# XuehaiPan/mate

Hardware: AMD Instinct MI355X
Metric: env-steps/sec MATE-4v8-9 batch=4096 per GPU (random policy, auto-reset) (higher is better)
Workload: dtype f64; 1 GPU; MATE-4v8-9.yaml batch=4096 envs per GPU, uniform random policy (on-device Philox), fused 256-step launches, restarts every 1 launch(es); global_batch=4096, parallelism=env-shard x1, steps_per_launch=256

## Files before the change

### mate_amd/csrc/device_math.hpp

```cpp
#pragma once
#include <hip/hip_runtime.h>
#include <stdint.h>

namespace mate {

constexpr double kRad2Deg = 180.0 / 3.14159265358979323846;
constexpr double kDeg2Rad = 3.14159265358979323846 / 180.0;
constexpr double kTerrain = 1000.0;
constexpr double kWarehouseRadius = 75.0;
constexpr double kWarehouseCenter = 925.0;
constexpr double kMaxViewingAngle = 180.0;

enum Stream : uint32_t { S_TRANSMIT = 1, S_GOAL = 2, S_ACT_CAM = 3, S_ACT_TGT = 4, S_RESET = 5, S_RESET_VIEW = 6 };

struct U4 { uint32_t x, y, z, w; };

__device__ __forceinline__ U4 philox(uint32_t k0, uint32_t k1, uint32_t c0, uint32_t c1, uint32_t c2, uint32_t c3) {
#pragma unroll
    for (int r = 0; r < 10; ++r) {
        const uint64_t p0 = (uint64_t)0xD2511F53u * c0;
        const uint64_t p1 = (uint64_t)0xCD9E8D57u * c2;
        const uint32_t n0 = (uint32_t)(p1 >> 32) ^ c1 ^ k0;
        const uint32_t n1 = (uint32_t)p1;
        const uint32_t n2 = (uint32_t)(p0 >> 32) ^ c3 ^ k1;
// ... 83 lines not shown
    p = FMA_SCX(p, z, 0xbf9e9ae6fc27006aull); p = FMA_SCX(p, z, 0x3fa2c15b5711927aull); p = FMA_SCX(p, z, 0xbfa59976e82d3ff0ull);
    p = FMA_SCX(p, z, 0x3fa82d5d6ef28734ull); p = FMA_SCX(p, z, 0xbfaae5ce6a214619ull); p = FMA_SCX(p, z, 0x3fae1bb48427b883ull);
    p = FMA_SCX(p, z, 0xbfb110e48b207f05ull); p = FMA_SCX(p, z, 0x3fb3b13657b87036ull); p = FMA_SCX(p, z, 0xbfb745d119378e4full);
    p = FMA_SCX(p, z, 0x3fbc71c717e1913cull); p = FMA_SCX(p, z, 0xbfc2492492376b7dull); p = FMA_SCX(p, z, 0x3fc99999999952ccull);
    p = FMA_SCX(p, z, 0xbfd5555555555523ull);
    double r = fma(t, z * p, t);
    const double half_pi = __longlong_as_double(0x3ff921fb54442d18ll), pi = __longlong_as_double(0x400921fb54442d18ll);
    if (ay > ax) r = half_pi - r;
    if (x < 0.0) r = pi - r;
    if (y == 0.0) r = x < 0.0 ? pi : 0.0;
    return copysign(r, y);
}
__device__ __forceinline__ double atan2_deg(double y, double x) { return atan2_finite(y, x) * kRad2Deg; }
__device__ __forceinline__ double atan2_sector(double y, double x) {
    const double ax = fabs(x), ay = fabs(y);
    const bool steep = ay > ax, back = x < 0.0;
    const double t = div_nz(steep ? ax : ay, steep ? ay : ax);
    const double z = t * t;
    double p = __longlong_as_double(0x3eeba404b5e68a13ll);
    p = FMA_SCX(p, z, 0xbf23e260bd3237f4ull); p = FMA_SCX(p, z, 0x3f4b2bb069efb384ull); p = FMA_SCX(p, z, 0xbf67952daf56de9bull);
    p = FMA_SCX(p, z, 0x3f7d6d43a595c56full); p = FMA_SCX(p, z, 0xbf8c6ea4a57d9582ull); p = FMA_SCX(p, z, 0x3f967e295f08b19full);
    p = FMA_SCX(p, z, 0xbf9e9ae6fc27006aull); p = FMA_SCX(p, z, 0x3fa2c15b5711927aull); p = FMA_SCX(p, z, 0xbfa59976e82d3ff0ull);
    p = FMA_SCX(p, z, 0x3fa82d5d6ef28734ull); p = FMA_SCX(p, z, 0xbfaae5ce6a214619ull); p = FMA_SCX(p, z, 0x3fae1bb48427b883ull);
    p = FMA_SCX(p, z, 0xbfb110e48b207f05ull); p = FMA_SCX(p, z, 0x3fb3b13657b87036ull); p = FMA_SCX(p, z, 0xbfb745d119378e4full);
    p = FMA_SCX(p, z, 0x3fbc71c717e1913cull); p = FMA_SCX(p, z, 0xbfc2492492376b7dull); p = FMA_SCX(p, z, 0x3fc99999999952ccull);
    p = FMA_SCX(p, z, 0xbfd5555555555523ull);
    const double r = fma(t, z * p, t);
    const uint32_t base_hi = steep ? 0x3ff921fbu : (back ? 0x400921fbu : 0u);
    const uint32_t base_lo = (steep || back) ? 0x54442d18u : 0u;
    const double base = __hiloint2double((int)base_hi, (int)base_lo);
    const uint32_t flip = (steep != back) ? 0x80000000u : 0u;
    const double sr = __hiloint2double(__double2hiint(r) ^ (int)flip, __double2loint(r));
    return copysign(base + sr, y);
}

__device__ __forceinline__ void sincos_deg(double deg, double &sn, double &cs) {
    const double x = deg * kDeg2Rad;
    const double k = rint(x * 0.63661977236758134308);
    double r = fma(-k, 1.57079632679489655800e+00, x);
    r = fma(-k, 6.12323399573676603587e-17, r);
    const double z = r * r;
    double ps = 2.81145725434552075980e-15;
    ps = FMA_SC(ps, z, -7.64716373181981647590e-13);
    ps = FMA_SC(ps, z, 1.60590438368216145994e-10);
    ps = FMA_SC(ps, z, -2.50521083854417187751e-08);
    ps = FMA_SC(ps, z, 2.75573192239858906526e-06);
    ps = FMA_SC(ps, z, -1.98412698412698412698e-04);
    ps = FMA_SC(ps, z, 8.33333333333333333333e-03);
    ps = FMA_SC(ps, z, -1.66666666666666666667e-01);
    const double s0 = fma(r * z, ps, r);
    double pc = -1.56192069685862264622e-16;
    pc = FMA_SC(pc, z, 4.77947733238738529744e-14);
    pc = FMA_SC(pc, z, -1.14707455977297247139e-11);
    pc = FMA_SC(pc, z, 2.08767569878680989792e-09);
    pc = FMA_SC(pc, z, -2.75573192239858906526e-07);
    pc = FMA_SC(pc, z, 2.48015873015873015873e-05);
    pc = FMA_SC(pc, z, -1.38888888888888888889e-03);
    pc = FMA_SC(pc, z, 4.16666666666666666667e-02);
    const double c0 = fma(z * z, pc, fma(-0.5, z, 1.0));
    const int q = (int)k & 3;
    const double sa = (q & 1) ? c0 : s0, ca = (q & 1) ? s0 : c0;
    sn = (q & 2) ? -sa : sa;
    cs = ((q + 1) & 2) ? -ca : ca;
}

__device__ __forceinline__ void sincos_deg_f32(double deg, float &sn, float &cs) {
// ... 66 lines not shown
```

### mate_amd/csrc/engine_kernels.hpp

```cpp
#pragma once
#include "device_math.hpp"
#include "instrument.hpp"

namespace mate {

enum Mode : int32_t { MODE_STEP = 0, MODE_STEP_RANDOM = 1, MODE_OBSERVE = 2 };

enum { TI_BOUNTY = 0, TI_FREIGHT = 1, TI_GW = 2, TI_TSTEPS = 3, TI_TRSTEPS = 4, TI_STRIDE = 5 };
enum { EI_REMAINING = 0, EI_AWAITING = 16, EI_DELIVERED = 20, EI_EPSTEP = 21, EI_TICK = 22, EI_EPISODE = 23, EI_DONE = 24, EI_PAD = 25, EI_COUNT = 26 };

struct Params {
    int32_t Nc, Nt, No, NK, NJ;
    int32_t Dc, Dt, cam_elems, tgt_elems;
    int32_t SW, DF, NI, DW;
    int32_t n_sector, n_range, sector_rounds, range_rounds;
    int32_t bit_cc, bit_range, bit_camobs, bit_always, MW;
    int32_t fs_range, fs_camobs, fs_always, fs_shared, nflags;
    int32_t nscratch, sc_cam, sc_tgt, sc_obs;
    int32_t tgt_table_off;
    int32_t kmax, nbucket;
    int32_t max_episode_steps, sparse_reward, num_cargoes_per_target, shuffle, start_with_cargoes, n_high;
    int32_t obs_f64;
    float inv_Nt, inv_NK, inv_NJ, inv_Nc;
    double tau, cam_radius, theta_min, rmax, rot, zoom, area, tgt_step, tgt_sight;
// ... 131 lines not shown
    float *scalars;
    uint32_t *masks;
    int32_t *idle_steps;
    uint32_t *own_masks;
    int32_t *done_count;
    int32_t *done_list;
    int32_t *flag_count;
    int32_t *flag_list;
    int32_t *lut_overflow;
    int32_t lut_defer_above;
    const uint8_t *reset_mask;
    const double *reset_tape;
    int32_t reset_tape_len;
    int32_t *reset_draws;
    double *ep_stats;
    double *sort_scratch;
    uint32_t *dev_tick_ptr;
    int32_t *ctrl;
    long long *phase_clocks;
    int32_t debug_skip;
    int64_t N;
    int32_t mode, act_f64, parity, reset_kind;
    int32_t rollout_steps;
    int32_t freeze_done;
    uint32_t tick;
    uint32_t tick_advance;
    int32_t stagger;
    const double2 *cam_grid, *tgt_grid;
    int32_t n_cam_grid, n_tgt_grid;
    int32_t act_discrete;
    int32_t obs_mode;
    int32_t rotate_prio;
    int32_t store_shifted;
    int32_t pipelined;
    int32_t per_step;
};
constexpr int32_t kDoneTag = 4;

__device__ __forceinline__ void phase_prio(int mode, int phase) {
    if (mode == 0) return;
    const int k = (mode >> (2 * phase)) & 3;
    if (k == 0) __builtin_amdgcn_s_setprio(0);
    else if (k == 1) __builtin_amdgcn_s_setprio(1);
    else if (k == 2) __builtin_amdgcn_s_setprio(2);
    else __builtin_amdgcn_s_setprio(3);
}

__device__ __forceinline__ const Ptrs &kernarg_ptrs(const Ptrs &g) {
    static_assert(alignof(Ptrs) == 8 && sizeof(const Params *) == 8, "g follows pp at byte 8 of the kernel arguments");
#if defined(__HIP_DEVICE_COMPILE__)
    (void)g;
    return *(const Ptrs *)((const char *)__builtin_amdgcn_kernarg_segment_ptr() + 8);
#else
    return g;
#endif
}

__device__ __forceinline__ void wave_sync() {
    __builtin_amdgcn_fence(__ATOMIC_RELEASE, "workgroup", "local");
    __builtin_amdgcn_wave_barrier();
    __builtin_amdgcn_fence(__ATOMIC_ACQUIRE, "workgroup", "local");
}

enum Flow : int {
    FLOW_ANY = 0,
    FLOW_RANDOM = 1,
// ... 520 lines not shown
    overflow = w[0].x != w[0].x;
    double2 k0 = w[0], k1 = w[1];
#pragma unroll
    for (int i = 1; i < kDegSlots - 1; ++i)
        if (w[i].x <= x) { k0 = w[i]; k1 = w[i + 1]; }
    if (k0.x == x) return k0.y;
    const double slope = (k1.y - k0.y) / (k1.x - k0.x);
    double res = slope * (x - k0.x) + k0.y;
    if (res != res) {
        res = slope * (x - k1.x) + k1.y;
        if (res != res && k0.y == k1.y) res = k0.y;
    }
    return res;
}

struct SectorEval { bool seen, need; double rn, x; int64_t lc; };

constexpr int kRoleRounds = 5;
__device__ __forceinline__ float range_rim(float lim) { return lim * (lim * 2e-5f + 2e-3f); }
template <typename ObsT, int L>
__device__ __forceinline__ bool range_exact(const Ctx<ObsT, L> &c, int tj, int j) {
    const double dx = c.ex[tj] - c.ex[j], dy = c.ey[tj] - c.ey[j];
    const double d2 = fma(dy, dy, dx * dx);
    const double lim = c.p.tgt_sight + c.er[j], lim2 = lim * lim;
    if (d2 < lim2 * (1.0 - 1e-14)) return true;
    if (d2 > lim2 * (1.0 + 1e-14)) return false;
    return sqrt_pos(d2) <= lim;
}
typedef __attribute__((address_space(3))) const double lds_cf64;
typedef __attribute__((address_space(3))) const float lds_cf32;
__device__ __forceinline__ uint32_t lds_addr(const void *q) { return (uint32_t)(uintptr_t)(__attribute__((address_space(3))) const char *)q; }
__device__ __forceinline__ double lds_f64(uint32_t a, int byte_off = 0) { return *(lds_cf64 *)(uintptr_t)(a + (uint32_t)byte_off); }
__device__ __forceinline__ float lds_f32(uint32_t a, int byte_off = 0) { return *(lds_cf32 *)(uintptr_t)(a + (uint32_t)byte_off); }
constexpr uint32_t kPass1Diag = 0xfffffffeu, kPass1None = 0xffffffffu;
constexpr int kSectorDiag = -3;
struct RangeRoles {
    uint32_t at[kRoleRounds], aj[kRoleRounds];
    float lim2[kRoleRounds];
    float rim[kRoleRounds];
    int32_t sector;
    uint32_t sec_cam, sec_other, sec_draw;
    uint32_t pass1[2];
    uint32_t block[1 + kRoleRounds];
    uint32_t block_bits;
    float reach2[kRoleRounds];
};
__device__ __forceinline__ void image_block_of(const Params &p, bool viewer_is_camera, int viewer, int j, uint32_t &word, uint32_t &code) {
    int src, col;
    if (j < p.Nc) { src = p.off_pub + 32 * j; code = 3u; }
    else if (j < p.Nc + p.No) { src = p.off_pub + 32 * (p.Nc + p.Nt) + 16 * (j - p.Nc); code = 1u; }
    else { src = p.off_pub + 32 * p.Nc + 32 * (j - p.Nc - p.No); code = 2u; }
    if (viewer_is_camera) {
        col = 22 + (j < p.Nc ? 5 * p.Nt + 4 * p.No + 7 * j : j < p.Nc + p.No ? 5 * p.Nt + 4 * (j - p.Nc) : 5 * (j - p.Nc - p.No));
        word = (uint32_t)src | ((uint32_t)(p.off_img + 4 * (viewer * p.Dc + col)) << 16);
    } else {
        col = 27 + (j < p.Nc ? 7 * j : j < p.Nc + p.No ? 7 * p.Nc + 4 * (j - p.Nc) : 7 * p.Nc + 4 * p.No + 5 * (j - p.Nc - p.No));
        word = (uint32_t)src | ((uint32_t)(p.off_img + 4 * (p.cam_elems + viewer * p.Dt + col)) << 16);
    }
}
__device__ __forceinline__ void pin_roles(RangeRoles &r, int rounds = kRoleRounds, bool image = true, bool sector = true) {
#pragma unroll
    for (int i = 0; i < kRoleRounds; ++i)
        if (i < rounds) { asm volatile("" : "+v"(r.at[i])); asm volatile("" : "+v"(r.aj[i])); asm volatile("" : "+v"(r.lim2[i])); asm volatile("" : "+v"(r.rim[i])); asm volatile("" : "+v"(r.reach2[i])); }
    if (image) {
#pragma unroll
        for (int i = 0; i < 1 + kRoleRounds; ++i)
            if (i <= rounds) asm volatile("" : "+v"(r.block[i]));
        asm volatile("" : "+v"(r.block_bits));
    }
    if (sector) { asm volatile("" : "+v"(r.sector)); asm volatile("" : "+v"(r.sec_cam)); asm volatile("" : "+v"(r.sec_other)); asm volatile("" : "+v"(r.sec_draw)); }
    else { asm volatile("" : "+v"(r.pass1[0])); asm volatile("" : "+v"(r.pass1[1])); }
}
template <typename ObsT>
__device__ __forceinline__ void range_roles(const Ctx<ObsT> &c, RangeRoles &roles) {
    const Params &p = c.p;
    roles.block_bits = 0;
    roles.sector = sector_role(p, (p.sector_rounds - 1) * 64 + c.lane);
#pragma unroll
    for (int round = 0; round < kRoleRounds; ++round) {
        const int q = round * 64 + c.lane;
        const int qq = q < p.n_range ? q : 0;
        const int t = (int)(((float)qq + 0.5f) * p.inv_NJ);
        const int j = qq - t * p.NJ;
        const int tj = c.tgt_slot(t);
        const float lim = (float)(p.tgt_sight + c.er[j]);
        const bool valid = q < p.n_range && round < p.range_rounds;
        roles.at[round] = lds_addr(c.exf + tj); roles.aj[round] = lds_addr(c.exf + j);
        roles.lim2[round] = !valid ? -INFINITY : j == tj ? INFINITY : lim * lim - range_rim(lim);
        roles.rim[round] = !valid ? -INFINITY : j == tj ? INFINITY : lim * lim + range_rim(lim);
        {
            const float step = (float)(((c.capword() >> t) & 1ull) ? p.tgt_step * 0.5 : p.tgt_step);
            const float reach = step + (float)c.er[j] + 1e-3f;
            roles.reach2[round] = (q < p.n_range && round < p.range_rounds && j < p.Nc + p.No) ? reach * reach : -1.0f;
        }
        roles.block[1 + round] = 0u;
        if (c.image() && q < p.n_range && round < p.range_rounds) {
            uint32_t code;
            image_block_of(p, false, t, j, roles.block[1 + round], code);
            roles.block_bits |= code << (2 * (1 + round));
        }
    }
#pragma unroll
    for (int round = 0; round < 2; ++round) {
        const int role = sector_role(p, round * 64 + c.lane);
        roles.pass1[round] = kPass1None;
        if (role >= 0) {
            const int cam = role & 0xff, other = (role >> 8) & 0xff;
            const bool is_target = (role >> 16) & 1;
            roles.pass1[round] = !is_target && cam == other ? kPass1Diag : (uint32_t)(8 * cam) | ((uint32_t)(8 * (is_target ? c.tgt_slot(other) : other)) << 16);
        }
    }
    roles.block[0] = 0u;
    roles.sec_cam = roles.sec_other = roles.sec_draw = lds_addr(c.base);
    if (roles.sector >= 0) {
        const int cam = roles.sector & 0xff, other = (roles.sector >> 8) & 0xff;
        const bool is_target = (roles.sector >> 16) & 1;
        const int oj = is_target ? c.tgt_slot(other) : other;
        if (c.image()) {
            uint32_t code;
            image_block_of(p, true, cam, oj, roles.block[0], code);
            roles.block_bits |= code;
        }
        roles.sec_cam += 8u * (uint32_t)cam; roles.sec_other += 8u * (uint32_t)oj;
        if (is_target) roles.sec_draw += 8u * (uint32_t)(cam * p.Nt + other);
        if (!is_target && cam == other) roles.sector = kSectorDiag;
    }
}

template <typename ObsT>
__device__ __forceinline__ void near_seed(const Ctx<ObsT> &c, const RangeRoles &roles, NearCarry &near) {
#pragma unroll
    for (int round = 0; round < kRoleRounds; ++round) {
        near.w[round] = 0ull;
        if (round < c.p.range_rounds) {
            const float dx = lds_f32(roles.at[round]) - lds_f32(roles.aj[round]);
            const float dy = lds_f32(roles.at[round], 4 * c.p.NJ) - lds_f32(roles.aj[round], 4 * c.p.NJ);
            near.w[round] = __ballot(fmaf(dy, dy, dx * dx) <= roles.reach2[round]);
        }
    }
}

__device__ __forceinline__ int sector_role(const Params &p, int q) {
    if (q < 0 || q >= p.n_sector) return -1;
    int cam, other; bool is_target;
    if (q < p.bit_cc) { cam = (int)(((float)q + 0.5f) * p.inv_Nt); other = q - cam * p.Nt; is_target = true; }
    else { const int r = q - p.bit_cc; cam = (int)(((float)r + 0.5f) * p.inv_Nc); other = r - cam * p.Nc; is_target = false; }
    return cam | (other << 8) | ((int)is_target << 16);
}
constexpr int kNoRole = -2;
__device__ __forceinline__ bool sector_out_of_range(double d2, double s2) {
    if (d2 > s2 * (1.0 + 1e-14)) return true;
    return !(d2 < s2 * (1.0 - 1e-14)) && sqrt_pos(d2) > sqrt_pos(s2);
}
template <bool RANGED = false, typename ObsT, int L>
__device__ __forceinline__ SectorEval sector_eval(Ctx<ObsT, L> &c, int q, uint32_t tick, uint32_t stream, bool predrawn, int role = kNoRole) {
    const Params &p = c.p;
// ... 27 lines not shown
}

template <typename ObsT>
__device__ __forceinline__ SectorEval sector_eval_held(Ctx<ObsT> &c, const RangeRoles &h, uint32_t tick, uint32_t stream, bool predrawn) {
    const Params &p = c.p;
    SectorEval e;
    e.seen = false; e.need = false;
    const int role = h.sector;
    if (role < 0) { e.seen = role == kSectorDiag; return e; }
    const int ent = p.off_ent, yoff = 8 * p.NJ;
    const double rx = lds_f64(h.sec_other, ent) - lds_f64(h.sec_cam, ent), ry = lds_f64(h.sec_other, ent + yoff) - lds_f64(h.sec_cam, ent + yoff);
    const double d2 = fma(ry, ry, rx * rx);
    if (sector_out_of_range(d2, lds_f64(h.sec_cam, p.off_tmp))) return e;
    const double ang = atan2_sector(ry, rx) * kRad2Deg;
    double ra = fabs(lds_f64(h.sec_cam, p.off_dy) - ang);
    const double alt = 360.0 - ra;
    if (alt < ra) ra = alt;
    if (ra * 2.0 > lds_f64(h.sec_cam, p.off_dy + 8 * p.Nc)) return e;
    if (p.No == 0) { e.seen = true; return e; }
    if ((role >> 16) & 1) {
        double u;
        if (predrawn && p.Nc * p.Nt <= c.predrawn_pairs()) u = lds_f64(h.sec_draw, p.off_tmp + 8 * (p.Nc + p.Nt));
        else {
            const int pair = (role & 0xff) * p.Nt + ((role >> 8) & 0xff);
            if (predrawn && pair < c.predrawn_pairs()) u = c.udraw(pair);
            else u = c.draw(tick, stream, (uint32_t)pair);
        }
        if ((p.tau <= 0.5) ? (u > 1.0 - p.tau) : (u <= p.tau)) { e.seen = true; return e; }
    }
    e.need = true; e.rn = d2; e.x = normalize_angle(ang); e.lc = c.env * p.Nc + (role & 0xff);
    return e;
}

template <typename ObsT, int L>
__device__ __forceinline__ void sector_fetch(const Ctx<ObsT, L> &c, const SectorEval &e, double2 (&w)[kDegWords]) {
    if (e.need) {
        const double2 *rec = c.g.lut_deg + (e.lc * kLutCells + degree_of(e.x)) * kDegWords;
#pragma unroll
        for (int i = 0; i < kDegWords; ++i) w[i] = rec[i];
    }
}

template <typename ObsT, int L>
__device__ __forceinline__ bool sector_resolve(const Ctx<ObsT, L> &c, const SectorEval &e, double2 (&w)[kDegWords]) {
    if (!e.need) return e.seen;
    bool overflow;
    double limit = segment_interp(w, e.x, overflow);
    if (overflow) {
        int start = (int)w[0].y, count = (int)w[1].x;
        const double2 *knots = c.g.lut_knots + e.lc * c.p.kmax;
        if (c.pivots && count >= 2 && count <= kPivotKnots && w[1].y > 0.0) {
            const int q = (int)w[1].y, last = count - 1;
            const double pv[8] = {w[2].x, w[2].y, w[3].x, w[3].y, w[4].x, w[4].y, w[5].x, w[5].y};
            int nle = 0;
#pragma unroll
            for (int i = 0; i < 8; ++i) nle += pv[i] <= e.x ? 1 : 0;
            const int base = nle * q;
#pragma unroll
            for (int i = 0; i < kDegSlots; ++i) w[i] = knots[start + (base + i < last ? base + i : last)];
            limit = degree_interp(w, e.x, overflow);
        } else {
        while (count > kQuarterKnots && count <= 4 * 256 + 1) {
            const int q = (count + 2) / 4, last = count - 1;
            const double a1 = knots[start + (q < last ? q : last)].x;
            const double a2 = knots[start + (2 * q < last ? 2 * q : last)].x;
            const double a3 = knots[start + (3 * q < last ? 3 * q : last)].x;
            const int base = e.x >= a3 ? 3 * q : (e.x >= a2 ? 2 * q : (e.x >= a1 ? q : 0));
            start += base;
            count = (q + 1 < count - base) ? q + 1 : count - base;
        }
        if (count >= 2 && count <= kQuarterKnots) {
            const int q = (count + 2) / 4, last = count - 1;
            const double a1 = knots[start + (q < last ? q : last)].x;
            const double a2 = knots[start + (2 * q < last ? 2 * q : last)].x;
            const double a3 = knots[start + (3 * q < last ? 3 * q : last)].x;
            const int base = e.x >= a3 ? 3 * q : (e.x >= a2 ? 2 * q : (e.x >= a1 ? q : 0));
#pragma unroll
            for (int i = 0; i < kDegSlots; ++i) w[i] = knots[start + (base + i < last ? base + i : last)];
            limit = degree_interp(w, e.x, overflow);
        } else {
            limit = lut_lookup(knots, c.g.lut_bucket + e.lc * c.p.nbucket, c.g.lut_count[e.lc], e.x);
        }
        }
    }
    const double lim = limit * (1.0 + 1e-6), lim2 = lim * lim;
    if (e.rn < lim2 * (1.0 - 1e-14)) return lim > 0.0;
    if (e.rn > lim2 * (1.0 + 1e-14)) return false;
    return sqrt_pos(e.rn) <= lim;
}

template <bool HELD, bool COMPACT = false, typename ObsT, int L>
__device__ __forceinline__ void update_view(Ctx<ObsT, L> &c, uint32_t tick, uint32_t stream, bool predrawn, const RangeRoles &held, uint32_t &seen_out,
                                            NearCarry *near_next = nullptr, unsigned long long *sector_ballot = nullptr) {
    const Params &p = c.p;
    const int lane = c.lane;
    seen_out = 0u;
    double2 w[kDegWords];
    int n_cand = 0;
    uint8_t *cand = c.base + p.off_list;
    static_assert(L == 64 || !HELD, "held lane roles: one wave per environment");
    const bool compact = L == 64 && COMPACT && p.sector_rounds >= 2 && p.n_sector <= 256;
#define MATE_N_SR (L == 64 ? p.sector_rounds : c.rounds_of(p.n_sector))
#define MATE_N_RR (L == 64 ? p.range_rounds : c.rounds_of(p.n_range))
    if (compact) {
        for (int round = 0; round < p.sector_rounds; ++round) {
            const int q = round * 64 + lane;
            bool diag = false, in_range = false;
            if (HELD && p.sector_rounds == 2) {
                const uint32_t held_pair = held.pass1[round & 1];
                if (held_pair != kPass1None) {
                    diag = held_pair == kPass1Diag;
                    if (!diag) {
                        const uint32_t a_cam = lds_addr(c.base) + (held_pair & 0xffffu), a_oj = lds_addr(c.base) + (held_pair >> 16);
                        const double rx = lds_f64(a_oj, p.off_ent) - lds_f64(a_cam, p.off_ent), ry = lds_f64(a_oj, p.off_ent + 8 * p.NJ) - lds_f64(a_cam, p.off_ent + 8 * p.NJ);
                        in_range = !sector_out_of_range(fma(ry, ry, rx * rx), lds_f64(a_cam, p.off_tmp));
                    }
                    set_flag(c, q, diag);
                }
            } else {
            const int role = sector_role(p, q);
            if (role >= 0) {
                const int cam = role & 0xff, other = (role >> 8) & 0xff;
                const bool is_target = (role >> 16) & 1;
                diag = !is_target && cam == other;
// ... 86 lines not shown
        write_range_ballots();
        if (lane < n_cand) {
            sector_fetch(c, first, w);
            if (sector_resolve(c, first, w)) { set_flag(c, q_first, true); atomicOr(&c.mask[q_first >> 5], 1u << (q_first & 31)); }
        }
        asm volatile("" :: "v"(touch0), "v"(touch1));
        for (int k = lane + 64; k < n_cand; k += 64) {
            const int q = cand[k];
            const SectorEval e = sector_eval<true>(c, q, tick, stream, predrawn);
            sector_fetch(c, e, w);
            if (sector_resolve(c, e, w)) { set_flag(c, q, true); atomicOr(&c.mask[q >> 5], 1u << (q & 31)); }
        }
    } else {
        const bool both_in_flight = L < 64 && MATE_N_SR == 2 && p.Nc * p.Nt < 16;
        SectorEval early;
        early.seen = false; early.need = false;
        double2 w_early[kDegWords];
        if (both_in_flight) {
            early = sector_eval(c, lane, tick, stream, predrawn);
            sector_fetch(c, early, w_early);
        }
        for (int round = 0; round + 1 < MATE_N_SR && !both_in_flight; ++round) {
            const SectorEval e = sector_eval(c, round * L + lane, tick, stream, predrawn);
            sector_fetch(c, e, w);
            const bool seen = sector_resolve(c, e, w);
            if (round * L + lane < p.n_sector) set_flag(c, round * L + lane, seen);
            const unsigned long long b = c.ballot(seen);
            if constexpr (L == 64) { if (lane == 0) { c.mask[2 * round] = (uint32_t)b; c.mask[2 * round + 1] = (uint32_t)(b >> 32); } }
            else c.put_bits(round * L, b);
        }
        const int last = MATE_N_SR - 1;
        SectorEval pending;
        pending.seen = false; pending.need = false;
        if (last >= 0) {
            if constexpr (HELD) pending = sector_eval_held(c, held, tick, stream, predrawn);
            else pending = sector_eval(c, last * L + lane, tick, stream, predrawn);
            sector_fetch(c, pending, w);
        }
        SUB_STAMP(c, 13);
        range_tests();
        if (both_in_flight) {
            const bool seen = sector_resolve(c, early, w_early);
            if (lane < p.n_sector) set_flag(c, lane, seen);
            c.put_bits(0, c.ballot(seen));
        }
        if (last >= 0) {
            const bool seen = sector_resolve(c, pending, w);
            if (!c.image() && last * L + lane < p.n_sector) set_flag(c, last * L + lane, seen);
            seen_out |= (uint32_t)seen;
            const unsigned long long b = c.ballot(seen);
            if constexpr (L == 64) { if (lane == 0) { c.mask[2 * last] = (uint32_t)b; c.mask[2 * last + 1] = (uint32_t)(b >> 32); } }
            else c.put_bits(last * L, b);
            if (sector_ballot) *sector_ballot = b;
        }
        write_range_ballots();
    }
    SUB_STAMP(c, 14);
    if (!c.statics_done) {
        if (lane < p.Nc) {
            const uint64_t m = c.camobs(lane);
            c.mask[(p.bit_camobs >> 5) + 2 * lane] = (uint32_t)m;
            c.mask[(p.bit_camobs >> 5) + 2 * lane + 1] = (uint32_t)(m >> 32);
        }
        if (lane == 0) { c.mask[p.bit_always >> 5] = 1u; if (!c.image()) set_flag(c, p.fs_always, true); }
        if (!c.image())
        for (int q = lane; q < p.Nc * p.No; q += L) {
            const int cam = (int)(((float)q + 0.5f) * p.inv_No);
            const int o = q - cam * p.No;
            set_flag(c, p.fs_camobs + cam * p.No + o, (c.camobs(cam) >> o) & 1ull);
        }
    }
    if (sector_ballot) return;
    wave_sync();
    if (lane < p.Nt) {
        int any = 0;
        for (int cam = 0; cam < p.Nc; ++cam) any |= (int)c.mask_bit(cam * p.Nt + lane);
        c.tracked(lane) = any;
        const double x = c.tx(lane), y = c.ty(lane);
        const bool px = x > 0.0, py = y > 0.0;
        const double wx = px ? kWarehouseCenter : -kWarehouseCenter, wy = py ? kWarehouseCenter : -kWarehouseCenter;
// ... 1241 lines not shown
    if (blockIdx.x == 0 && threadIdx.x == 0 && g.done_count) g.done_count[g.parity ^ 1] = 0;
    const int wave = __builtin_amdgcn_readfirstlane((int)(threadIdx.x >> 6));
    const int hw_lane = threadIdx.x & 63, lane = hw_lane & (L - 1), shift = hw_lane & ~(L - 1);
    const int slot = E == 1 ? wave : wave * E + (hw_lane >> (E == 8 ? 3 : E == 4 ? 4 : 5));
    const int64_t env = (int64_t)blockIdx.x * (4 * E) + slot;
    if (env >= g.N) return;
    const Ptrs &gk = kernarg_ptrs(g);
    MATE_PROF(const long long t_wave = (long long)__builtin_amdgcn_s_memtime();)
    {
        Ctx<ObsT, L> c(p, gk, smem + slot * p.lds_wave_bytes, lane, env, FLOW_ANY, shift);
        load_records(c);
        wave_sync();
        build_entities(c);
        if (!(E > 1 && g.per_step && !g.freeze_done)) list_finished_at_entry(c);
        wave_sync();
    }
    PROLOGUE_STAMP(8);
    constexpr bool IMAGE = E == 1 && Shape::kImage;
    constexpr bool HOLD_ROLES = E == 1 && Shape::kHoldRoles;
    static_assert(E == 1 || !Shape::kImage, "the row image is a whole-wave mode");
    static_assert(kNearWords == kRoleRounds, "one ballot per range round");
    static_assert(!IMAGE || (Shape::kHoldRoles && sizeof(ObsT) == 4 && FLOW != FLOW_ANY), "row-image mode: f32 rows, held lane roles, a folded flow");
    constexpr int kSubC = (Shape::kChunksC + L - 1) / L, kSubT = (Shape::kChunksT + L - 1) / L;
    constexpr int kGC = E == 1 ? Shape::kHeldGC : (kSubC + kSubT <= 12 ? kSubC : 2), kGT = E == 1 ? Shape::kHeldGT : (kSubC + kSubT <= 12 ? kSubT : 6);
    PackDescriptorsT<kGC, kGT> held;
    if constexpr (!IMAGE) {
        Ctx<ObsT, L> c(p, gk, smem + slot * p.lds_wave_bytes, lane, env, FLOW, shift);
        load_pack_descriptors(c, held);
    }
    RangeRoles roles;
    if constexpr (HOLD_ROLES) {
        Ctx<ObsT> c(p, gk, smem + wave * p.lds_wave_bytes, lane, env, FLOW);
        range_roles(c, roles);
        pin_roles(roles);
        PROLOGUE_STAMP(9);
        if constexpr (IMAGE) image_statics(c);
    }
    PROLOGUE_STAMP(10);
    NearCarry near{};
    if constexpr (HOLD_ROLES) {
        Ctx<ObsT> c(p, gk, smem + wave * p.lds_wave_bytes, lane, env, FLOW);
        near_seed(c, roles, near);
    }
    uint32_t hw_id;
    asm volatile("s_getreg_b32 %0, hwreg(HW_REG_HW_ID)" : "=s"(hw_id));
    const int wave_slot = (int)(hw_id & 15u);
    MATE_PROF(long long acc[8] = {0, 0, 0, 0, 0, 0, 0, 0};
              long long t_prev = (long long)__builtin_amdgcn_s_memtime();
              const long long t_first = t_prev, r_first = (long long)__builtin_amdgcn_s_memrealtime();)
    bool stepped = false;
    int last_gw = -1;
    DrawCarry carry{0u, 0u, 0xffffffffu};
    DrawRole draws_of_lane;
    {
        Ctx<ObsT, L> c(p, gk, smem + slot * p.lds_wave_bytes, lane, env, FLOW, shift);
        draws_of_lane = draw_role(c);
    }
    constexpr bool HELDSTATE = IMAGE && FLOW == FLOW_RANDOM;
    HeldState h{};
    int finished = 0;
    const uint32_t tick0 = (E > 1 ? p.dev_tick : 0u) + g.tick;
    const uint32_t cam_low = (uint32_t)(reinterpret_cast<uintptr_t>(g.cam_obs) >> 4) & 7u, tgt_low = (uint32_t)(reinterpret_cast<uintptr_t>(g.tgt_obs) >> 4) & 7u;
    const int n_steps = g.rollout_steps;
    if constexpr (HELDSTATE) {
        Ctx<ObsT> c(p, gk, smem + wave * p.lds_wave_bytes, lane, env, FLOW);
        held_load(c, h);
        finished = __builtin_amdgcn_readfirstlane((int)(c.ei(EI_DONE) != 0));
    }
    PROLOGUE_STAMP(11);
#pragma clang loop unroll(disable)
    for (int r = 0; r < n_steps; ++r) {
        int lane_r = lane, wave_r = wave, slot_r = slot;
        asm volatile("" : "+v"(lane_r));
        asm volatile("" : "+s"(wave_r));
        if constexpr (E == 1) slot_r = wave_r; else asm volatile("" : "+v"(slot_r));
        const Params *pr = pp;
        asm volatile("" : "+s"(pr));
        const Shape shape_r(pr, true);
        const Params &p = shape_r.get();
        const int64_t env_r = (int64_t)blockIdx.x * (4 * E) + slot_r;
        if constexpr (HOLD_ROLES) pin_roles(roles, p.range_rounds, IMAGE, p.sector_rounds == 1);
        Ctx<ObsT, L> c(p, gk, smem + slot_r * p.lds_wave_bytes, lane_r, env_r, FLOW, shift);
        c.out = (int64_t)r * g.N + env_r;
        c.statics_done = stepped;
        c.pivots = Shape::kGreedyHeld;
        if (HELDSTATE ? finished != 0 : (c.ei(EI_DONE) != 0 && (E == 1 || !g.per_step || g.freeze_done))) {
            if (lane_r == 0 && g.scalars) { float *o = g.scalars + c.out * 8; o[0] = 0.f; o[1] = 0.f; o[2] = 2.f; o[3] = o[4] = o[5] = o[6] = o[7] = 0.f; }
            if (lane_r == 0 && g.idle_steps) g.idle_steps[env_r] += 1;
            continue;
        }
        const uint32_t tick = tick0 + (uint32_t)r;
        if (g.rotate_prio) {
            const int turn = g.rotate_prio >= 8 ? ((int)(__builtin_amdgcn_s_memtime() >> g.rotate_prio) + wave_slot) & 3 : (r + wave_slot) & 3;
            if (turn & 2) { if (turn & 1) __builtin_amdgcn_s_setprio(3); else __builtin_amdgcn_s_setprio(2); }
            else { if (turn & 1) __builtin_amdgcn_s_setprio(1); else __builtin_amdgcn_s_setprio(0); }
        }
        ROLL_STAMP(7);
        StepDraws draws{0.0, 0.0};
        pin_draw_role(draws_of_lane);
        draws = step_draws(c, tick, &carry, &draws_of_lane);
        if constexpr (FLOW == FLOW_ACT_F32) draws = prefetch_action(c);
        ROLL_STAMP(0);
        if constexpr (HELDSTATE) {
            simulate_cameras_held(c, draws, h);
            ROLL_STAMP(1);
            simulate_targets_held(c, draws, near, h);
            ROLL_STAMP(2);
            uint32_t seen = 0u;
            unsigned long long sector_ballot = 0ull;
            update_view<true, true>(c, tick, S_TRANSMIT, true, roles, seen, &near, &sector_ballot);
            bool tracked; int inside;
            view_tail_held(c, sector_ballot, h, tracked, inside);
            ROLL_STAMP(3);
            finished = assign_and_score_held(c, tick, g.scalars, h, tracked, inside);
            ROLL_STAMP(4);
            image_targets_held(c, h, last_gw); image_blocks(c, roles, seen);
            ROLL_STAMP(5);
            image_store(c, cam_low, tgt_low); store_masks(c);
            wave_sync();
            stepped = true;
            ROLL_STAMP(6);
            continue;
        }
        simulate_cameras(c, draws, true);
        ROLL_STAMP(1);
        simulate_targets(c, draws, HOLD_ROLES ? &near : nullptr);
        ROLL_STAMP(2);
        uint32_t seen = 0u;
        update_view<HOLD_ROLES, true>(c, tick, S_TRANSMIT, true, roles, seen, HOLD_ROLES ? &near : nullptr);
        ROLL_STAMP(3);
        assign_and_score(c, tick, g.scalars);
        ROLL_STAMP(4);
        if constexpr (IMAGE) {
            image_targets(c, last_gw); image_blocks(c, roles, seen);
            ROLL_STAMP(5);
            image_store(c, cam_low, tgt_low); store_masks(c);
        } else {
            fill_scratch(c, last_gw);
            ROLL_STAMP(5);
            pack_observations<true, Shape::kGreedyHeld>(c, held);
        }
        wave_sync();
        stepped = true;
// ... 23 lines not shown
```

### mate_amd/csrc/mate_engine.hip

```cpp
#include <hip/hip_runtime.h>
#include <hip/hip_ext.h>

#include <algorithm>
#include <atomic>
#include <cmath>
#include <cstdarg>
#include <cstdio>
#include <cstdlib>
#include <cstring>
#include <map>
#include <mutex>
#include <random>
#include <string>
#include <vector>

#include "../../include/mate_engine.h"
#include "reset_kernels.hpp"
#include "policy_kernels.hpp"
#include "aux_kernels.hpp"
#include "state_rows.hpp"

using namespace mate;

static thread_local std::string g_error;
// ... 31 lines not shown
#include "shape_group.inc"
#undef MATE_SHAPE_GROUP
#define MATE_SHAPE_GROUP 5
#include "shape_group.inc"
#undef MATE_SHAPE_GROUP
#endif

static KernelSet pick_kernels(int Nc, int Nt, int No, bool f64, bool generic, bool no_image) {
    KernelSet k;
    if (!generic && (pick_kernels_group0(Nc, Nt, No, f64, no_image, &k) || pick_kernels_group1(Nc, Nt, No, f64, no_image, &k) ||
                     pick_kernels_group2(Nc, Nt, No, f64, no_image, &k) || pick_kernels_group3(Nc, Nt, No, f64, no_image, &k) ||
                     pick_kernels_group4(Nc, Nt, No, f64, no_image, &k) || pick_kernels_group5(Nc, Nt, No, f64, no_image, &k))) {
        k.specialised = 1;
        return k;
    }
    return f64 ? f64_kernels<AnyShape>() : f32_kernels<AnyShape, void, true>(no_image);
}

struct Switches {
    bool generic = false;
    bool flow_generic = false;
    int stagger = -1;
    int lut_small_cap = 0;
    bool reset_monolithic = false;
    int rollout_rotate = 1;
    bool no_image = false;
    bool policy_split = false;
    int step_split = -1;
    bool zoom_iterate = false;
    bool step_sub_wave = true;
    int sub_wave_mode = 2;
    bool step_greedy_rollout = false;
    bool pipelined_low_priority = true;
    bool pipelined_serial = false;
};
static Switches read_switches() {
    Switches w;
    auto flag = [](const char *name) { const char *v = getenv(name); return v && atoi(v) != 0; };
    w.generic = flag("MATE_GENERIC");
    w.flow_generic = flag("MATE_FLOW_GENERIC");
    if (const char *v = getenv("MATE_STAGGER")) w.stagger = atoi(v);
    if (const char *v = getenv("MATE_LUT_SMALL_CAP")) w.lut_small_cap = atoi(v);
    w.reset_monolithic = flag("MATE_RESET_MONOLITHIC");
    if (const char *v = getenv("MATE_ROLLOUT_ROTATE")) w.rollout_rotate = atoi(v);
    w.zoom_iterate = flag("MATE_ZOOM_ITERATE");
    w.policy_split = flag("MATE_POLICY_SPLIT");
    w.step_greedy_rollout = flag("MATE_STEP_GREEDY_ROLLOUT");
    w.no_image = flag("MATE_NO_IMAGE");
    if (const char *v = getenv("MATE_STEP_SUBWAVE")) w.step_sub_wave = atoi(v) != 0;
    if (const char *v = getenv("MATE_SUBWAVE")) w.sub_wave_mode = atoi(v) == 0 ? 0 : 1;
    if (const char *v = getenv("MATE_STEP_SPLIT")) w.step_split = atoi(v) != 0;
    if (const char *v = getenv("MATE_PIPELINED_PRIORITY")) w.pipelined_low_priority = atoi(v) != 0;
    w.pipelined_serial = flag("MATE_PIPELINED_SERIAL");
    return w;
}

struct mate_engine {
    Switches sw{};
    hipStream_t last_stream = nullptr;
    bool launched = false, multi_stream = false;
    Params p{};
    Params *d_params = nullptr;
    Ptrs g{};
    ResetLds rl{};
    ResetLds rl_small{};
    mate_config cfg{};
    int device = 0;
    int64_t N = 0;
    int parity = 0;
    uint32_t tick = 0;
    int64_t steps_since_reset = 0;
    bool was_reset = false;
    bool dev_tick = false;
    int dev_frames = 1;
    int dev_interval = 1;
    int pending_interval = 0;
    bool pipelined = false;
    int pipe_every = 1, pipe_count = 0;
    hipStream_t side = nullptr;
    hipEvent_t ev_launch = nullptr, ev_reset[2] = {nullptr, nullptr};
    bool reset_in_flight[2] = {false, false};
    size_t step_lds = 0, reset_lds = 0;
    KernelSet k{};
    size_t image_wave_bytes = 0;
    int64_t cus = 256;
    int split_on = 0;
// ... 798 lines not shown
    HIP_TRY(hipGetLastError());
    if (mode == MODE_OBSERVE) return MATE_OK;
    if (!e->dev_tick) e->tick += 1;
    return restart_finished(e, auto_reset, Restart{io, true, RESET_DONE, PH_PLACE | PH_LUT | PH_VIEW, false, e->greedy_team_bits != 0, 1u, kStepFlow}, stream);
}

extern "C" int mate_engine_step(mate_engine *e, const mate_step_io *io, int32_t auto_reset, void *stream) {
    return refresh_state_rows(e, launch_step(e, io, MODE_STEP, auto_reset, (hipStream_t)stream), stream);
}
extern "C" int mate_engine_step_random(mate_engine *e, const mate_step_io *io, int32_t auto_reset, void *stream) {
    return refresh_state_rows(e, launch_step(e, io, MODE_STEP_RANDOM, auto_reset, (hipStream_t)stream), stream);
}
static int sub_wave_of_launch(const mate_engine *e, bool greedy) {
    const int mode = e->sw.sub_wave_mode;
    if (mode == 0 || e->k.sub_wave <= 1 || !(greedy ? (const void *)e->k.rollout_greedy_sub : (const void *)e->k.rollout_sub[0])) return 1;
    if (mode == 1) return e->k.sub_wave;
    if (e->N < 32 * e->cus) return 1;
    if (!greedy && e->p.Nc * e->p.Nt >= 16) return 1;
    return e->k.sub_wave;
}

static int rollout_random_impl(mate_engine *e, const mate_step_io *io, int32_t steps, int32_t auto_reset, void *stream_) {
    if (!e) return fail(MATE_EINVAL, "null engine");
    hipStream_t stream = (hipStream_t)stream_;
    { const int rc_ = enter(e, stream, "rollout"); if (rc_ != MATE_OK) return rc_; }
    if (e->dev_tick) return fail(MATE_ESTATE, "not available while the step counter is device-resident (mate_engine_device_tick)");
    if (steps < 1) return fail(MATE_EINVAL, "rollout needs at least one step");
    note_stream(e, stream);
    { int rc = flush_pending(e, auto_reset, kRolloutFlow, stream); if (rc != MATE_OK) return rc; }
    Ptrs g = e->g;
    apply_io(g, io);
    g.mode = MODE_STEP_RANDOM; g.parity = e->parity; g.reset_kind = -1; g.tick = e->tick; g.rollout_steps = steps;
    g.tape_ct = nullptr; g.tape_goal = nullptr;
    g.rotate_prio = e->sw.rollout_rotate;
    if (auto_reset != 1) g.done_count = nullptr;
    const int E = sub_wave_of_launch(e, false);
    const unsigned blocks = (unsigned)((e->N + 4 * E - 1) / (4 * E));
    Timed t;
    { const int rc_ = take_timing_events(e, true, &t); if (rc_ != MATE_OK) return rc_; }
    const int flow = (!e->sw.flow_generic && !g.act_discrete && g.obs_mode == 0 && !g.xdesc && !g.xab && g.scratch_init &&
                      (g.cam_obs || e->p.Nc == 0) && g.tgt_obs && g.scalars) ? FLOW_RANDOM : FLOW_ANY;
    e->last_flow = flow;
    const StepFn fn = E > 1 ? e->k.rollout_sub[flow] : e->k.rollout[flow];
    const size_t lds = E > 1 ? E * e->step_lds : (flow == FLOW_RANDOM && e->k.image) ? 4 * e->image_wave_bytes : e->step_lds;
    hipExtLaunchKernelGGL(fn, dim3(blocks), dim3(256), lds, stream, t.a, t.b, 0, (const Params *)e->d_params, (const Ptrs)g);
    HIP_TRY(hipGetLastError());
    e->tick += (uint32_t)steps;
    return restart_finished(e, auto_reset, Restart{nullptr, false, RESET_FLAGGED, PH_PLACE | PH_LUT, false, false, 0u, kRolloutFlow}, stream);
}

extern "C" int mate_engine_rollout_random(mate_engine *e, const mate_step_io *io, int32_t steps, int32_t auto_reset, void *stream) {
    return refresh_state_rows(e, rollout_random_impl(e, io, steps, auto_reset, stream), stream);
}

static size_t fused_rollout_lds(const mate_engine *e, int E = 1) { return (size_t)E * (4 * (size_t)e->p.lds_wave_bytes + 4 * (size_t)policy_slice_bytes(e->q.PW, e->p.Nc, e->p.Nt)) + (E == 1 ? 1024 : 0); }
static size_t step_greedy_lds(const mate_engine *e, bool cameras = true) {
    return 4 * (size_t)e->p.lds_wave_bytes + 4 * (size_t)step_greedy_slice_bytes(e->q.PW, e->q.TW, e->p.Nc, e->p.Nt, e->p.MW, cameras);
}
static bool use_step_greedy(const mate_engine *e) { return e->k.step_greedy && !e->sw.step_greedy_rollout && step_greedy_lds(e) <= 160 * 1024; }

static int policy_enable(mate_engine *e) {
    if (e->policy_ready) return MATE_OK;
    const Params &p = e->p;
    PolicyPtrs &q = e->q;
    q.TW = pol_target_words(p.Nt);
    q.PW = pol_record_words(p.Nc, p.Nt);
    q.caller_team = -1;
// ... 117 lines not shown
            int least = 0, greatest = 0;
            HIP_TRY(hipDeviceGetStreamPriorityRange(&least, &greatest));
            if (!e->sw.pipelined_low_priority) HIP_TRY(hipStreamCreateWithFlags(&e->side, hipStreamNonBlocking));
            else HIP_TRY(hipStreamCreateWithPriority(&e->side, hipStreamNonBlocking, least));
        }
        HIP_TRY(hipEventCreateWithFlags(&e->ev_launch, hipEventDisableTiming));
        for (int q = 0; q < 2; ++q) HIP_TRY(hipEventCreateWithFlags(&e->ev_reset[q], hipEventDisableTiming));
    }
    if (pipelined && !e->pipelined) {
        HIP_TRY(hipMemsetAsync(e->g.done_count, 0, 2 * sizeof(int32_t), stream));
        e->reset_in_flight[0] = e->reset_in_flight[1] = false;
        e->pipelined = true;
        e->pipe_every = pipe_every; e->pipe_count = 0;
    }
    Ptrs g = e->g;
    apply_io(g, io);
    g.pipelined = pipelined ? 1 : 0;
    if ((e->p.Nc > 0 && !g.cam_obs) || !g.tgt_obs || !g.scalars) return fail(MATE_EINVAL, "rollout_greedy needs the observation and scalar outputs");
    if (g.obs_mode != 0 || g.xdesc) return fail(MATE_EINVAL, "rollout_greedy packs plain observations (no fused transform / team mode)");
    if (team_caller == 0 && e->p.Nc == 0) return fail(MATE_EINVAL, "the scenario has no cameras to act for");
    if (team_caller >= 0 && !(team_caller == 0 ? g.cam_act : g.tgt_act))
        return fail(MATE_EINVAL, "rollout_versus_greedy needs the %s team's joint action", team_caller == 0 ? "camera" : "target");
    if (team_caller >= 0 && (((g.act_discrete & 1) && team_caller == 0 && !g.cam_grid) || ((g.act_discrete & 2) && team_caller == 1 && !g.tgt_grid)))
        return fail(MATE_ESTATE, "discrete actions passed before mate_engine_set_action_grids");
    const int E = ((!per_step || e->sw.step_sub_wave) && fused_rollout_lds(e, e->k.sub_wave) <= 160 * 1024) ? sub_wave_of_launch(e, true) : 1;
    const bool light = per_step && use_step_greedy(e) && E == 1;
    const PolicyFn fn = light ? e->k.step_greedy : E > 1 ? e->k.rollout_greedy_sub : e->k.rollout_greedy;
    const size_t lds = light ? step_greedy_lds(e, team_caller != 0) : fused_rollout_lds(e, E);
    if (lds > 160 * 1024) return fail(MATE_EINVAL, "rollout_greedy: %zu bytes of LDS per workgroup do not fit", lds);
    g.mode = MODE_STEP; g.reset_kind = -1; g.rollout_steps = steps;
    g.parity = e->dev_tick ? 0 : e->parity;
    g.tick = e->dev_tick ? (uint32_t)e->steps_since_reset * (uint32_t)steps : e->tick;
    g.tape_ct = nullptr; g.tape_goal = nullptr; g.freeze_done = 0;
    g.rotate_prio = e->sw.rollout_rotate;
    if (per_step ? auto_reset == 0 : (auto_reset != 1 && !pipelined)) g.done_count = nullptr;
    if (pipelined && e->reset_in_flight[e->parity]) { HIP_TRY(hipStreamWaitEvent(stream, e->ev_reset[e->parity], 0)); e->reset_in_flight[e->parity] = false; }
    PolicyPtrs q = e->q;
    std::memset(&q.tape, 0, sizeof(q.tape));
    q.caller_team = team_caller;
    const unsigned blocks = (unsigned)((e->N + 4 * E - 1) / (4 * E));
    Timed t;
    { const int rc_ = take_timing_events(e, !e->dev_tick, &t); if (rc_ != MATE_OK) return rc_; }
    e->last_flow = light ? FLOW_STEP_GREEDY : FLOW_GREEDY;
    launch(fn, dim3(blocks), dim3(256), lds, stream, t, e->d_params, g, q);
    HIP_TRY(hipGetLastError());
    if (!e->dev_tick) e->tick += (uint32_t)steps;
    const int full = PH_PLACE | PH_LUT | PH_VIEW;
    if (per_step) return restart_finished(e, auto_reset, Restart{io, false, RESET_DONE, full, false, true, 1u, kStepFlow}, stream);
    if (!pipelined) return restart_finished(e, auto_reset, Restart{nullptr, false, RESET_FLAGGED, full, true, false, (uint32_t)steps, kRolloutFlow}, stream);
    if (++e->pipe_count < e->pipe_every) return MATE_OK;
    e->pipe_count = 0;
    const bool serial = e->sw.pipelined_serial;
    hipStream_t rs = serial ? stream : e->side;
    if (!serial) { HIP_TRY(hipEventRecord(e->ev_launch, stream)); HIP_TRY(hipStreamWaitEvent(rs, e->ev_launch, 0)); }
    Ptrs r = restart_ptrs(e);
    r.pipelined = 1;
    const bool multi_before = e->multi_stream;
    int rc = launch_reset(e, r, RESET_DONE, full, rs, true);
    if (rc != MATE_OK) return rc;
    HIP_TRY(hipMemsetAsync(e->g.done_count + e->parity, 0, sizeof(int32_t), rs));
    if (!serial) { HIP_TRY(hipEventRecord(e->ev_reset[e->parity], rs)); e->reset_in_flight[e->parity] = true; }
    e->last_stream = stream; e->multi_stream = multi_before;
    e->parity ^= 1;
    return MATE_OK;
}

extern "C" int mate_engine_rollout_greedy(mate_engine *e, const mate_step_io *io, int32_t steps, int32_t auto_reset, void *stream) {
// ... 479 lines not shown
```

Measured before the change: 765.8 million env-steps/s.

## Add f32 screening pass for sector visibility with exact f64 fallback on band

Adds a float32 pre-screen for the camera sector visibility test. It uses fast rsq/rcp, an f32 atan2 and tolerance bands to classify each pair as seen, hidden or needing the LUT cell, and runs the exact f64 sector evaluation only when some lane in the wave lands inside an uncertainty band. The aim is to cut f64 atan2/sqrt work and LUT recomputation in the held-roles rollout path. It needs extra pinned registers for the pass1 LDS addresses and adds wave-wide ballots. It also depends on the band margins being wide enough to keep results exact. The path is compiled only when MATE_SECTOR_SCREEN is defined and can be disabled at runtime with MATE_SECTOR_EXACT.

```diff
diff --git a/mate_amd/csrc/device_math.hpp b/mate_amd/csrc/device_math.hpp
--- a/mate_amd/csrc/device_math.hpp
+++ b/mate_amd/csrc/device_math.hpp
@@ -139,6 +139,57 @@
     const uint32_t flip = (steep != back) ? 0x80000000u : 0u;
     const double sr = __hiloint2double(__double2hiint(r) ^ (int)flip, __double2loint(r));
     return copysign(base + sr, y);
+}
+
+constexpr float kSectorShift = 1.74e-4f;
+#if defined(__HIP_DEVICE_COMPILE__)
+__host__ __device__ __forceinline__ float rsq_f32(float x) { return __builtin_amdgcn_rsqf(x); }
+__host__ __device__ __forceinline__ float rcp_f32(float x) { return __builtin_amdgcn_rcpf(x); }
+#else
+__host__ __device__ __forceinline__ float rsq_f32(float x) { return 1.0f / __builtin_sqrtf(x); }
+__host__ __device__ __forceinline__ float rcp_f32(float x) { return 1.0f / x; }
+#endif
+__host__ __device__ __forceinline__ float atan2_deg_f32(float y, float x) {
+    const float ax = __builtin_fabsf(x), ay = __builtin_fabsf(y);
+    const bool steep = ay > ax, back = x < 0.0f;
+    const float t = (steep ? ax : ay) * rcp_f32(steep ? ay : ax);
+    const float z = t * t;
+    float p = 0.0073740179650485516f;
+    p = __builtin_fmaf(p, z, -0.03551992028951645f); p = __builtin_fmaf(p, z, 0.08216780424118042f); p = __builtin_fmaf(p, z, -0.13398802280426025f);
+    p = __builtin_fmaf(p, z, 0.1986185610294342f); p = __builtin_fmaf(p, z, -0.3332539498806f);
+    const float r = __builtin_fmaf(t, z * p, t) * 57.29577951308232f;
+    const float base = steep ? 90.0f : (back ? 180.0f : 0.0f);
+    const float a = (steep != back) ? base - r : base + r;
+    return __builtin_copysignf(a, y);
+}
+__host__ __device__ __forceinline__ float sector_bearing_band(float inv_d) { return __builtin_fmaf(1.25e-2f, inv_d, 2e-4f); }
+__host__ __device__ __forceinline__ int sector_range_screen(float d2f, float df, float s2f) {
+    const float band = __builtin_fmaf(8e-4f, df, __builtin_fmaf(1e-6f, d2f + s2f, 1e-6f));
+    const float diff = d2f - s2f;
+    return diff > band ? 1 : (diff < -band ? -1 : 0);
+}
+__host__ __device__ __forceinline__ int sector_angle_screen(float bearing, float phif, float thetaf, float band) {
+    float ra = __builtin_fabsf(phif - bearing);
+    const float alt = 360.0f - ra;
+    if (alt < ra) ra = alt;
+    const float over = __builtin_fmaf(2.0f, ra, -thetaf), rim = __builtin_fmaf(2.0f, band, 4e-4f);
+    return over > rim ? 1 : (over < -rim ? -1 : 0);
+}
+__host__ __device__ __forceinline__ bool sector_cell_screen(float bearing, float band, int cells_per_degree, int &cell) {
+    const float u = (bearing + 180.0f) * (float)cells_per_degree;
+    const float fl = __builtin_floorf(u), fr = u - fl, rim = __builtin_fmaf((float)cells_per_degree, band, 1e-4f);
+    int c = (int)fl;
+    const int last = 360 * cells_per_degree - 1;
+    c = c < 0 ? 0 : (c > last ? last : c);
+    cell = c;
+    return fr > rim && 1.0f - fr > rim;
+}
+__host__ __device__ __forceinline__ int sector_limit_screen(float df, float limf, float slopef, float lead, float band) {
+    const float lim = limf * 1.000001f;
+    const float rim = __builtin_fmaf(__builtin_fabsf(slopef), band, __builtin_fmaf(1e-6f, df + limf, 4e-4f));
+    if (!(lead >= band)) return 0;
+    const float diff = df - lim;
+    return diff > rim ? 1 : (diff < -rim ? -1 : 0);
 }
 
 __device__ __forceinline__ void sincos_deg(double deg, double &sn, double &cs) {
diff --git a/mate_amd/csrc/engine_kernels.hpp b/mate_amd/csrc/engine_kernels.hpp
--- a/mate_amd/csrc/engine_kernels.hpp
+++ b/mate_amd/csrc/engine_kernels.hpp
@@ -187,6 +187,7 @@
     int32_t obs_mode;
     int32_t rotate_prio;
     int32_t store_shifted;
+    int32_t sector_exact;
     int32_t pipelined;
     int32_t per_step;
 };
@@ -773,6 +774,11 @@
 __device__ __forceinline__ uint32_t lds_addr(const void *q) { return (uint32_t)(uintptr_t)(__attribute__((address_space(3))) const char *)q; }
 __device__ __forceinline__ double lds_f64(uint32_t a, int byte_off = 0) { return *(lds_cf64 *)(uintptr_t)(a + (uint32_t)byte_off); }
 __device__ __forceinline__ float lds_f32(uint32_t a, int byte_off = 0) { return *(lds_cf32 *)(uintptr_t)(a + (uint32_t)byte_off); }
+#if defined(MATE_SECTOR_SCREEN)
+constexpr bool kSectorScreen = true;
+#else
+constexpr bool kSectorScreen = false;
+#endif
 constexpr uint32_t kPass1Diag = 0xfffffffeu, kPass1None = 0xffffffffu;
 constexpr int kSectorDiag = -3;
 struct RangeRoles {
@@ -799,6 +805,7 @@
         word = (uint32_t)src | ((uint32_t)(p.off_img + 4 * (p.cam_elems + viewer * p.Dt + col)) << 16);
     }
 }
+template <bool SHADOW = false>
 __device__ __forceinline__ void pin_roles(RangeRoles &r, int rounds = kRoleRounds, bool image = true, bool sector = true) {
 #pragma unroll
     for (int i = 0; i < kRoleRounds; ++i)
@@ -811,6 +818,9 @@
     }
     if (sector) { asm volatile("" : "+v"(r.sector)); asm volatile("" : "+v"(r.sec_cam)); asm volatile("" : "+v"(r.sec_other)); asm volatile("" : "+v"(r.sec_draw)); }
     else { asm volatile("" : "+v"(r.pass1[0])); asm volatile("" : "+v"(r.pass1[1])); }
+    if constexpr (SHADOW) {
+        if (sector) { asm volatile("" : "+v"(r.pass1[0])); asm volatile("" : "+v"(r.pass1[1])); }
+    }
 }
 template <typename ObsT>
 __device__ __forceinline__ void range_roles(const Ctx<ObsT> &c, RangeRoles &roles) {
@@ -863,6 +873,7 @@
             roles.block_bits |= code;
         }
         roles.sec_cam += 8u * (uint32_t)cam; roles.sec_other += 8u * (uint32_t)oj;
+        if (kSectorScreen && c.image()) { roles.pass1[0] = lds_addr(c.base) + 4u * (uint32_t)cam; roles.pass1[1] = lds_addr(c.base) + 4u * (uint32_t)oj; }
         if (is_target) roles.sec_draw += 8u * (uint32_t)(cam * p.Nt + other);
         if (!is_target && cam == other) roles.sector = kSectorDiag;
     }
@@ -956,13 +967,66 @@
     return e;
 }
 
+enum : int { kScreenHidden = 0, kScreenSeen = 1, kScreenNeed = 2, kScreenBand = 3 };
+struct SectorScreen { int state; float df, bearing, half; int cell; };
+template <typename ObsT>
+__device__ __forceinline__ SectorScreen sector_screen_held(Ctx<ObsT> &c, const RangeRoles &h, uint32_t tick, uint32_t stream, bool predrawn) {
+    const Params &p = c.p;
+    SectorScreen s;
+    s.state = kScreenHidden;
+    const int role = h.sector;
+    if (role < 0) { s.state = role == kSectorDiag ? kScreenSeen : kScreenHidden; return s; }
+    const int entf = p.off_ent + 24 * p.NJ, yoff = 4 * p.NJ;
+    const float rx = lds_f32(h.pass1[1], entf) - lds_f32(h.pass1[0], entf), ry = lds_f32(h.pass1[1], entf + yoff) - lds_f32(h.pass1[0], entf + yoff);
+    const float d2 = fmaf(ry, ry, rx * rx);
+    const float inv_d = rsq_f32(d2), d = d2 * inv_d;
+    const int beyond = sector_range_screen(d2, d, (float)lds_f64(h.sec_cam, p.off_tmp));
+    if (beyond != -1) { s.state = beyond == 0 ? kScreenBand : kScreenHidden; return s; }
+    const float half = sector_bearing_band(inv_d), bearing = atan2_deg_f32(ry, rx);
+    const int outside = sector_angle_screen(bearing, (float)lds_f64(h.sec_cam, p.off_dy), (float)lds_f64(h.sec_cam, p.off_dy + 8 * p.Nc), half);
+    if (outside != -1) { s.state = outside == 0 ? kScreenBand : kScreenHidden; return s; }
+    if (p.No == 0) { s.state = kScreenSeen; return s; }
+    if ((role >> 16) & 1) {
+        double u;
+        if (predrawn && p.Nc * p.Nt <= c.predrawn_pairs()) u = lds_f64(h.sec_draw, p.off_tmp + 8 * (p.Nc + p.Nt));
+        else {
+            const int pair = (role & 0xff) * p.Nt + ((role >> 8) & 0xff);
+            if (predrawn && pair < c.predrawn_pairs()) u = c.udraw(pair);
+            else u = c.draw(tick, stream, (uint32_t)pair);
+        }
+        if ((p.tau <= 0.5) ? (u > 1.0 - p.tau) : (u <= p.tau)) { s.state = kScreenSeen; return s; }
+    }
+    s.state = sector_cell_screen(bearing, half, kCellsPerDegree, s.cell) ? kScreenNeed : kScreenBand;
+    s.df = d; s.bearing = bearing; s.half = half;
+    return s;
+}
+__device__ __forceinline__ bool sector_resolve_screened(const SectorScreen &s, const double2 (&w)[kDegWords], bool &band) {
+    band = false;
+    if (s.state != kScreenNeed) return s.state == kScreenSeen;
+    const double x = (double)s.bearing, xh = (double)(s.bearing + s.half);
+    const double xa = w[0].x, ya = w[0].y, sa = w[1].x, xb = w[1].y, yb = w[2].x, sb = w[2].y;
+    const double xc = w[3].x, yc = w[3].y, sc = w[4].x, xd = w[4].y, yd = w[5].x, sd = w[5].y;
+    double x0 = xa, y0 = ya, sl = sa;
+    if (xb <= xh) { x0 = xb; y0 = yb; sl = sb; }
+    if (xc <= xh) { x0 = xc; y0 = yc; sl = sc; }
+    if (xd <= xh) { x0 = xd; y0 = yd; sl = sd; }
+    const double lead = x - x0;
+    const int hidden = sector_limit_screen(s.df, (float)(sl * lead + y0), (float)sl, (float)lead, s.half);
+    band = xa != xa || hidden == 0;
+    return hidden == -1;
+}
+
+template <typename ObsT, int L>
+__device__ __forceinline__ void sector_fetch_cell(const Ctx<ObsT, L> &c, bool need, int64_t lc, int cell, double2 (&w)[kDegWords]) {
+    if (need) {
+        const double2 *rec = c.g.lut_deg + (lc * kLutCells + cell) * kDegWords;
+#pragma unroll
+        for (int i = 0; i < kDegWords; ++i) w[i] = rec[i];
+    }
+}
 template <typename ObsT, int L>
 __device__ __forceinline__ void sector_fetch(const Ctx<ObsT, L> &c, const SectorEval &e, double2 (&w)[kDegWords]) {
-    if (e.need) {
-        const double2 *rec = c.g.lut_deg + (e.lc * kLutCells + degree_of(e.x)) * kDegWords;
-#pragma unroll
-        for (int i = 0; i < kDegWords; ++i) w[i] = rec[i];
-    }
+    if (e.need) sector_fetch_cell(c, true, e.lc, degree_of(e.x), w);
 }
 
 template <typename ObsT, int L>
@@ -1013,7 +1077,7 @@
     return sqrt_pos(e.rn) <= lim;
 }
 
-template <bool HELD, bool COMPACT = false, typename ObsT, int L>
+template <bool HELD, bool COMPACT = false, bool SCREEN = false, typename ObsT, int L>
 __device__ __forceinline__ void update_view(Ctx<ObsT, L> &c, uint32_t tick, uint32_t stream, bool predrawn, const RangeRoles &held, uint32_t &seen_out,
                                             NearCarry *near_next = nullptr, unsigned long long *sector_ballot = nullptr) {
     const Params &p = c.p;
@@ -1166,10 +1230,25 @@
         const int last = MATE_N_SR - 1;
         SectorEval pending;
         pending.seen = false; pending.need = false;
+        bool exact = true;
+        SectorScreen screened;
+        screened.state = kScreenHidden;
         if (last >= 0) {
-            if constexpr (HELD) pending = sector_eval_held(c, held, tick, stream, predrawn);
-            else pending = sector_eval(c, last * L + lane, tick, stream, predrawn);
-            sector_fetch(c, pending, w);
+            if constexpr (HELD && SCREEN) {
+                static_assert(L == 64, "the screen reads held lane roles");
+                if (!c.g.sector_exact) {
+                    screened = sector_screen_held(c, held, tick, stream, predrawn);
+                    exact = __ballot(screened.state == kScreenBand) != 0ull;
+                }
+                if (exact) { pending = sector_eval_held(c, held, tick, stream, predrawn); sector_fetch(c, pending, w); }
+                else sector_fetch_cell(c, screened.state == kScreenNeed, c.env * p.Nc + (held.sector & 0xff), screened.cell, w);
+            } else if constexpr (HELD) {
+                pending = sector_eval_held(c, held, tick, stream, predrawn);
+                sector_fetch(c, pending, w);
+            } else {
+                pending = sector_eval(c, last * L + lane, tick, stream, predrawn);
+                sector_fetch(c, pending, w);
+            }
         }
         SUB_STAMP(c, 13);
         range_tests();
@@ -1179,7 +1258,19 @@
             c.put_bits(0, c.ballot(seen));
         }
         if (last >= 0) {
-            const bool seen = sector_resolve(c, pending, w);
+            bool seen = false;
+            if constexpr (HELD && SCREEN) {
+                if (!exact) {
+                    bool band;
+                    seen = sector_resolve_screened(screened, w, band);
+                    if (__ballot(band) != 0ull) {
+                        exact = true;
+                        pending = sector_eval_held(c, held, tick, stream, predrawn);
+                        sector_fetch(c, pending, w);
+                    }
+                }
+            }
+            if (exact) seen = sector_resolve(c, pending, w);
             if (!c.image() && last * L + lane < p.n_sector) set_flag(c, last * L + lane, seen);
             seen_out |= (uint32_t)seen;
             const unsigned long long b = c.ballot(seen);
@@ -2487,7 +2578,7 @@
     if constexpr (HOLD_ROLES) {
         Ctx<ObsT> c(p, gk, smem + wave * p.lds_wave_bytes, lane, env, FLOW);
         range_roles(c, roles);
-        pin_roles(roles);
+        pin_roles<IMAGE && kSectorScreen>(roles, kRoleRounds, true, true);
         PROLOGUE_STAMP(9);
         if constexpr (IMAGE) image_statics(c);
     }
@@ -2534,7 +2625,7 @@
         const Shape shape_r(pr, true);
         const Params &p = shape_r.get();
         const int64_t env_r = (int64_t)blockIdx.x * (4 * E) + slot_r;
-        if constexpr (HOLD_ROLES) pin_roles(roles, p.range_rounds, IMAGE, p.sector_rounds == 1);
+        if constexpr (HOLD_ROLES) pin_roles<IMAGE && kSectorScreen>(roles, p.range_rounds, IMAGE, p.sector_rounds == 1);
         Ctx<ObsT, L> c(p, gk, smem + slot_r * p.lds_wave_bytes, lane_r, env_r, FLOW, shift);
         c.out = (int64_t)r * g.N + env_r;
         c.statics_done = stepped;
@@ -2563,7 +2654,7 @@
             ROLL_STAMP(2);
             uint32_t seen = 0u;
             unsigned long long sector_ballot = 0ull;
-            update_view<true, true>(c, tick, S_TRANSMIT, true, roles, seen, &near, &sector_ballot);
+            update_view<true, true, kSectorScreen>(c, tick, S_TRANSMIT, true, roles, seen, &near, &sector_ballot);
             bool tracked; int inside;
             view_tail_held(c, sector_ballot, h, tracked, inside);
             ROLL_STAMP(3);
diff --git a/mate_amd/csrc/mate_engine.hip b/mate_amd/csrc/mate_engine.hip
--- a/mate_amd/csrc/mate_engine.hip
+++ b/mate_amd/csrc/mate_engine.hip
@@ -87,6 +87,7 @@
     int sub_wave_mode = 2;
     bool step_greedy_rollout = false;
     bool pipelined_low_priority = true;
+    bool sector_exact = false;
     bool pipelined_serial = false;
 };
 static Switches read_switches() {
@@ -107,6 +108,7 @@
     if (const char *v = getenv("MATE_STEP_SPLIT")) w.step_split = atoi(v) != 0;
     if (const char *v = getenv("MATE_PIPELINED_PRIORITY")) w.pipelined_low_priority = atoi(v) != 0;
     w.pipelined_serial = flag("MATE_PIPELINED_SERIAL");
+    w.sector_exact = flag("MATE_SECTOR_EXACT");
     return w;
 }
 
@@ -971,7 +973,7 @@
     apply_io(g, io);
     g.mode = MODE_STEP_RANDOM; g.parity = e->parity; g.reset_kind = -1; g.tick = e->tick; g.rollout_steps = steps;
     g.tape_ct = nullptr; g.tape_goal = nullptr;
-    g.rotate_prio = e->sw.rollout_rotate;
+    g.rotate_prio = e->sw.rollout_rotate; g.sector_exact = e->sw.sector_exact ? 1 : 0;
     if (auto_reset != 1) g.done_count = nullptr;
     const int E = sub_wave_of_launch(e, false);
     const unsigned blocks = (unsigned)((e->N + 4 * E - 1) / (4 * E));
@@ -1155,7 +1157,7 @@
     g.parity = e->dev_tick ? 0 : e->parity;
     g.tick = e->dev_tick ? (uint32_t)e->steps_since_reset * (uint32_t)steps : e->tick;
     g.tape_ct = nullptr; g.tape_goal = nullptr; g.freeze_done = 0;
-    g.rotate_prio = e->sw.rollout_rotate;
+    g.rotate_prio = e->sw.rollout_rotate; g.sector_exact = e->sw.sector_exact ? 1 : 0;
     if (per_step ? auto_reset == 0 : (auto_reset != 1 && !pipelined)) g.done_count = nullptr;
     if (pipelined && e->reset_in_flight[e->parity]) { HIP_TRY(hipStreamWaitEvent(stream, e->ev_reset[e->parity], 0)); e->reset_in_flight[e->parity] = false; }
     PolicyPtrs q = e->q;
```

Result: slower. 746.8 million env-steps/s (-2.5%).
